# BDMstudio/audio-cut

Measured on AMD Instinct MI355X. Metric: audio-seconds processed/sec (separate+detect) per GPU; cut-point index parity, higher is better.
Workload: dtype f32

## Files before the change

### audio_cut_amd/csrc/ac_gemm.hip

```cpp
#include "ac_common.h"
#include "../../include/audiocut_hip_final.h"

typedef __attribute__((ext_vector_type(8))) _Float16 f16x8;
typedef __attribute__((ext_vector_type(4))) float f32x4;

#define GM_BM 128
#define GM_BM_FINAL 96
#define GM_BK 32
#define GM_ASTRIDE 48

__device__ inline unsigned short gm_f16_bits(_Float16 h) { return __builtin_bit_cast(unsigned short, h); }

template <int NT, bool RESID, int BM = GM_BM, int TR = 8, bool FINAL = false>
__global__ __launch_bounds__(256, 2) void k_tdf_linear_f16x3(const float* __restrict__ x, const f16x8* __restrict__ wpk,
                                                             const float* __restrict__ scale, const float* __restrict__ shift,
                                                             const float* __restrict__ resid, float* __restrict__ y,
                                                             int n_mblk, int N, int K, int T, int C, float w_unscale,
                                                             const float* __restrict__ in_amax, float* __restrict__ out_amax,
                                                             int ord_g, int ord_r, const float* __restrict__ fin_w = nullptr,
                                                             const float* __restrict__ fin_b = nullptr, float* __restrict__ spec = nullptr,
                                                             int C_out = 0) {
    static_assert(FINAL ? (BM == 96 && NT == 6 && RESID) : (BM == 128 && TR == 8), "row tiles: 16 channels x 8 time rows, or 48 x 2 with the final 1x1 conv");
    constexpr int MT = BM / 32;
    constexpr int A_ITERS = (BM * (GM_BK / 4)) / 256;
    constexpr int CH = BM / TR;
    constexpr int BN = 32 * NT;
    constexpr int BFRAGS = 2 * (BN / 16) * 64;
    constexpr int B_ITERS = BFRAGS / 256;
    constexpr int OSTRIDE = 16 * NT + 4;
    constexpr int A_BYTES = 2 * BM * GM_ASTRIDE * 2;
    constexpr int O_BYTES = 4 * 16 * OSTRIDE * 4;
    constexpr int TSTRIDE = BN + 4;
    constexpr int K_ARENA = A_BYTES + 2 * BFRAGS * 16, E_ARENA = FINAL ? BM * TSTRIDE * 4 : O_BYTES;
    constexpr int ARENA = K_ARENA > E_ARENA ? K_ARENA : E_ARENA;
    __shared__ __attribute__((aligned(16))) unsigned char s_raw[ARENA];
    unsigned short* s_hi = reinterpret_cast<unsigned short*>(s_raw);
    unsigned short* s_lo = s_hi + BM * GM_ASTRIDE;
    f16x8* s_b0 = reinterpret_cast<f16x8*>(s_raw + A_BYTES);
    f16x8* s_b1 = s_b0 + BFRAGS;
    float* s_out = reinterpret_cast<float*>(s_raw);

    const int tid = threadIdx.x, lane = tid & 63, wave = tid >> 6;
    const int wm = wave >> 1, wn = wave & 1;
    const int n_nblk = N / BN;
    int wi = blockIdx.x;
    if ((gridDim.x & 7) == 0) wi = (blockIdx.x & 7) * (gridDim.x >> 3) + (blockIdx.x >> 3);
    const int per = ord_r * n_nblk;
    const int chunk = wi / per, i_in = wi - chunk * per;
    const int nb_hi = i_in / (ord_g * ord_r), j_in = i_in - nb_hi * (ord_g * ord_r);
    const int nb = nb_hi * ord_g + j_in % ord_g, mb = chunk * ord_r + j_in / ord_g;
    if (mb >= n_mblk) return;
    const int n0 = nb * BN;
    const int n_stage = K / GM_BK;
    const int n_blk = T / TR, n_cg = C / CH;
    const int tb = mb % n_blk, cg = (mb / n_blk) % n_cg, item = mb / (n_blk * n_cg);
    const size_t m_base = ((size_t)item * C + (size_t)cg * CH) * T + (size_t)tb * TR;
    auto grow = [&](int r) -> size_t { return m_base + (size_t)(r / TR) * T + (r % TR); };
    __shared__ float s_scale[TR], s_inv[TR];
    __shared__ unsigned s_tmax[TR];
    if (tid < TR) {
        float inv;
        s_scale[tid] = ac_act_scale_lane(in_amax ? in_amax + (size_t)item * T : nullptr, tb * TR + tid, tb * TR + tid, &inv);
        s_inv[tid] = inv;
        s_tmax[tid] = 0u;
    }

    f32x4 acc[MT][NT];
#pragma unroll
    for (int m = 0; m < MT; ++m)
#pragma unroll
        for (int n = 0; n < NT; ++n) acc[m][n] = (f32x4){0.f, 0.f, 0.f, 0.f};

    const float* a_ptr[A_ITERS];
    int a_off[A_ITERS];
#pragma unroll
    for (int i = 0; i < A_ITERS; ++i) {
        const int e = tid + 256 * i;
        const int row = e >> 3, kq = e & 7;
        a_ptr[i] = x + grow(row) * (size_t)K + 4 * kq;
        a_off[i] = row * GM_ASTRIDE + 4 * kq;
    }
    const f16x8* wbase = wpk + (size_t)nb * n_stage * BFRAGS;

    float4 pre_a[A_ITERS];
    auto prefetch = [&](int s) {
        f16x8* dst = (s & 1) ? s_b1 : s_b0;
#pragma unroll
        for (int i = 0; i < B_ITERS; ++i) {
            const int inst = wave + 4 * i;
            __builtin_amdgcn_global_load_lds(wbase + (size_t)s * BFRAGS + inst * 64 + lane, dst + inst * 64, 16, 0, 0);
        }
#pragma unroll
        for (int i = 0; i < A_ITERS; ++i) pre_a[i] = *reinterpret_cast<const float4*>(a_ptr[i] + (size_t)s * GM_BK);
    };
    prefetch(0);
    __syncthreads();
    float a_scale[A_ITERS];
#pragma unroll
    for (int i = 0; i < A_ITERS; ++i) a_scale[i] = s_scale[((tid + 256 * i) >> 3) % TR];

    const int frag_row = lane & 15, frag_k = 8 * (lane >> 4);
    for (int s = 0; s < n_stage; ++s) {
        __syncthreads();
        const f16x8* s_b = (s & 1) ? s_b1 : s_b0;
#pragma unroll
        for (int i = 0; i < A_ITERS; ++i) {
            const float v[4] = {pre_a[i].x, pre_a[i].y, pre_a[i].z, pre_a[i].w};
            unsigned short h[4], l[4];
#pragma unroll
            for (int q = 0; q < 4; ++q) {
                const float c = fminf(fmaxf(v[q] * a_scale[i], -65504.f), 65504.f);
                const _Float16 hv = (_Float16)c;
                h[q] = gm_f16_bits(hv);
                l[q] = gm_f16_bits((_Float16)(c - (float)hv));
            }
            *reinterpret_cast<uint2*>(&s_hi[a_off[i]]) = make_uint2((unsigned)h[0] | ((unsigned)h[1] << 16), (unsigned)h[2] | ((unsigned)h[3] << 16));
            *reinterpret_cast<uint2*>(&s_lo[a_off[i]]) = make_uint2((unsigned)l[0] | ((unsigned)l[1] << 16), (unsigned)l[2] | ((unsigned)l[3] << 16));
        }
        __builtin_amdgcn_s_waitcnt(0);
        __syncthreads();
        if (s + 1 < n_stage) prefetch(s + 1);
        f16x8 ah[MT], al[MT];
#pragma unroll
        for (int m = 0; m < MT; ++m) {
            const int off = (wm * (BM / 2) + m * 16 + frag_row) * GM_ASTRIDE + frag_k;
            ah[m] = *reinterpret_cast<const f16x8*>(&s_hi[off]);
            al[m] = *reinterpret_cast<const f16x8*>(&s_lo[off]);
        }
#pragma unroll
        for (int n = 0; n < NT; ++n) {
            const f16x8 bh = s_b[(0 * (BN / 16) + wn * NT + n) * 64 + lane];
            const f16x8 bl = s_b[(1 * (BN / 16) + wn * NT + n) * 64 + lane];
#pragma unroll
            for (int m = 0; m < MT; ++m) {
                acc[m][n] = __builtin_amdgcn_mfma_f32_16x16x32_f16(ah[m], bl, acc[m][n], 0, 0, 0);
                acc[m][n] = __builtin_amdgcn_mfma_f32_16x16x32_f16(al[m], bh, acc[m][n], 0, 0, 0);
                acc[m][n] = __builtin_amdgcn_mfma_f32_16x16x32_f16(ah[m], bh, acc[m][n], 0, 0, 0);
            }
        }
    }
    if constexpr (FINAL) {
        constexpr int WR = BM / 2, WC = BN / 2;
        constexpr int ROW_F4 = WC / 4;
        constexpr int P_ITERS = 16 * ROW_F4 / 64;
        const int g = lane >> 4, px = lane & 15;
        float* s_tile = reinterpret_cast<float*>(s_raw);
        float* sw = s_tile + wm * WR * TSTRIDE + wn * WC;
        auto y_offset = [&](int m, int i, int& tr) -> size_t {
            const int e = lane + 64 * i;
            const int row = e / ROW_F4, q4 = e - row * ROW_F4;
            tr = wm * WR + m * 16 + row;
            return grow(tr) * (size_t)N + n0 + wn * WC + 4 * q4;
        };
        float4 rr[2][P_ITERS];
#pragma unroll
        for (int i = 0; i < P_ITERS; ++i) { int tr; rr[0][i] = *reinterpret_cast<const float4*>(resid + y_offset(0, i, tr)); }
        __syncthreads();
#pragma unroll
        for (int m = 0; m < MT; ++m)
#pragma unroll
            for (int n = 0; n < NT; ++n)
#pragma unroll
                for (int r = 0; r < 4; ++r) sw[(m * 16 + g * 4 + r) * TSTRIDE + n * 16 + px] = acc[m][n][r];
        __builtin_amdgcn_wave_barrier();
#pragma unroll
        for (int m = 0; m < MT; ++m) {
            if (m + 1 < MT) {
#pragma unroll
                for (int i = 0; i < P_ITERS; ++i) { int tr; rr[(m + 1) & 1][i] = *reinterpret_cast<const float4*>(resid + y_offset(m + 1, i, tr)); }
            }
#pragma unroll
            for (int i = 0; i < P_ITERS; ++i) {
                const int e = lane + 64 * i;
                const int row = e / ROW_F4, q4 = e - row * ROW_F4;
                int tr;
                const size_t o = y_offset(m, i, tr);
                const int c = cg * CH + tr / TR;
                const float sc = scale[c] * (w_unscale * s_inv[tr % TR]), sh = shift[c];
                float4* cell = reinterpret_cast<float4*>(&sw[(m * 16 + row) * TSTRIDE + 4 * q4]);
                float4 v = *cell;
                v.x = fmaxf(v.x * sc + sh, 0.f); v.y = fmaxf(v.y * sc + sh, 0.f);
                v.z = fmaxf(v.z * sc + sh, 0.f); v.w = fmaxf(v.w * sc + sh, 0.f);
                const float4 q = rr[m & 1][i];
                v.x += q.x; v.y += q.y; v.z += q.z; v.w += q.w;
                *cell = v;
                if (y) *reinterpret_cast<float4*>(y + o) = v;
            }
        }
        __syncthreads();
        if (tid < TR * (BN / 2)) {
            const int t = tid / (BN / 2), cp = tid - t * (BN / 2);
            const float* tp = s_tile + t * TSTRIDE + 2 * cp;
            int cw[4];
            float2 a[4];
#pragma unroll
            for (int co = 0; co < 4; ++co) {
                cw[co] = co < C_out ? co : 0;
                const float bv = fin_b[cw[co]];
                a[co] = make_float2(bv, bv);
            }
#pragma unroll
            for (int c = 0; c < CH; ++c) {
                const float2 v = *reinterpret_cast<const float2*>(tp + c * TR * TSTRIDE);
#pragma unroll
                for (int co = 0; co < 4; ++co) {
                    const float wv = fin_w[cw[co] * CH + c];
                    a[co].x = fmaf(wv, v.x, a[co].x); a[co].y = fmaf(wv, v.y, a[co].y);
                }
            }
#pragma unroll
            for (int co = 0; co < 4; ++co)
                if (co < C_out)
                    *reinterpret_cast<float2*>(spec + (((size_t)item * C_out + co) * T + (size_t)tb * TR + t) * N + n0 + 2 * cp) = a[co];
        }
        return;
    }
    const int g = lane >> 4, px = lane & 15;
    float* so = s_out + wave * 16 * OSTRIDE;
    constexpr int ROW_F4 = 4 * NT;
    constexpr int E_ITERS = 16 * ROW_F4 / 64;
    float4 rr[2][E_ITERS];
    auto out_offset = [&](int m, int i, int& c) -> size_t {
        const int e = lane + 64 * i;
        const int row = e / ROW_F4, q4 = e - row * ROW_F4;
        const int tr = wm * 64 + m * 16 + row;
        c = cg * 16 + (tr >> 3);
        return grow(tr) * (size_t)N + n0 + wn * (16 * NT) + 4 * q4;
    };
    if (RESID) {
#pragma unroll
        for (int i = 0; i < E_ITERS; ++i) { int c; rr[0][i] = *reinterpret_cast<const float4*>(resid + out_offset(0, i, c)); }
    }
    __syncthreads();
    float vm[E_ITERS];
#pragma unroll
    for (int i = 0; i < E_ITERS; ++i) vm[i] = 0.f;
#pragma unroll
    for (int m = 0; m < MT; ++m) {
#pragma unroll
        for (int n = 0; n < NT; ++n)
#pragma unroll
            for (int r = 0; r < 4; ++r) so[(g * 4 + r) * OSTRIDE + n * 16 + px] = acc[m][n][r];
        if (RESID && m + 1 < MT) {
#pragma unroll
            for (int i = 0; i < E_ITERS; ++i) { int c; rr[(m + 1) & 1][i] = *reinterpret_cast<const float4*>(resid + out_offset(m + 1, i, c)); }
        }
        __builtin_amdgcn_wave_barrier();
#pragma unroll
        for (int i = 0; i < E_ITERS; ++i) {
            const int e = lane + 64 * i;
            const int row = e / ROW_F4, q4 = e - row * ROW_F4;
            int c;
            const size_t o = out_offset(m, i, c);
            const int tr = wm * 64 + m * 16 + row;
            const float sc = scale[c] * (w_unscale * s_inv[tr & 7]), sh = shift[c];
            float4 v = *reinterpret_cast<const float4*>(&so[row * OSTRIDE + 4 * q4]);
            v.x = fmaxf(v.x * sc + sh, 0.f); v.y = fmaxf(v.y * sc + sh, 0.f);
            v.z = fmaxf(v.z * sc + sh, 0.f); v.w = fmaxf(v.w * sc + sh, 0.f);
            if (RESID) { const float4 q = rr[m & 1][i]; v.x += q.x; v.y += q.y; v.z += q.z; v.w += q.w; }
            vm[i] = fmaxf(fmaxf(vm[i], fmaxf(fabsf(v.x), fabsf(v.y))), fmaxf(fabsf(v.z), fabsf(v.w)));
            *reinterpret_cast<float4*>(y + o) = v;
        }
        __builtin_amdgcn_wave_barrier();
    }
    if (out_amax) {
#pragma unroll
        for (int i = 0; i < E_ITERS; ++i) {
            float a = fmaxf(vm[i], __shfl_xor(vm[i], 1, AC_WAVE));
            a = fmaxf(a, __shfl_xor(a, 2, AC_WAVE));
            if ((lane & 3) == 0) atomicMax(&s_tmax[((lane + 64 * i) / ROW_F4) & 7], __float_as_uint(a));
        }
        __syncthreads();
        if (tid < 8 && s_tmax[tid]) atomicMax(reinterpret_cast<unsigned*>(out_amax + (size_t)item * T + tb * 8 + tid), s_tmax[tid]);
    }
}

extern "C" int ac_tdf_linear_f16x3(ac_ctx* ctx, const float* x, const void* w_packed, const float* scale, const float* shift,
                                    const float* resid, float* y, long long M, int N, int K, int T, int C, float w_unscale,
                                    const float* in_amax, float* out_amax, void* stream) {
    AC_REQUIRE(ctx && x && w_packed && scale && shift && y, "null pointer");
    AC_REQUIRE(M > 0 && C > 0 && T > 0 && C % 16 == 0 && T % 8 == 0 && M % ((long long)C * T) == 0,
               "rows = items x C x T with C % 16 == 0 and T % 8 == 0 (a tile is 16 channels x 8 time rows)");
    AC_REQUIRE(K > 0 && K % GM_BK == 0, "K % 32 == 0");
    AC_REQUIRE(N > 0 && N % 96 == 0, "N % 96 == 0");
    const bool wide = (N % 192) == 0;
    const long long n_mblk = M / GM_BM;
    const int n_nblk = N / (wide ? 192 : 96);
    long long nblk = n_mblk * n_nblk;
    AC_REQUIRE(nblk < (1LL << 31) - 8 && n_mblk < (1LL << 31), "grid too large");
    int ord_g = n_nblk, ord_r = 1;
    if (n_nblk % 4 == 0 && n_nblk > 4 && n_mblk % 16 == 0) { ord_g = 4; ord_r = 16; }
    dim3 grid((unsigned)nblk), block(256);
    hipStream_t st = (hipStream_t)stream;
    const f16x8* wp = (const f16x8*)w_packed;
#define GM_GO(NT_, RES_) hipLaunchKernelGGL((k_tdf_linear_f16x3<NT_, RES_>), grid, block, 0, st, x, wp, scale, shift, resid, y, (int)n_mblk, N, K, T, C, w_unscale, in_amax, out_amax, ord_g, ord_r)
    if (wide) { if (resid) GM_GO(6, true); else GM_GO(6, false); }
    else      { if (resid) GM_GO(3, true); else GM_GO(3, false); }
#undef GM_GO
    AC_LAUNCH_CHECK();
    return AC_OK;
}

extern "C" int ac_tdf_linear_final_f16x3(ac_ctx* ctx, const float* x, const void* w_packed, const float* scale, const float* shift,
                                          const float* resid, const float* final_w, const float* final_b, float* spec, float* y,
                                          long long M, int N, int K, int T, int C, int C_out, float w_unscale, const float* in_amax,
                                          void* stream) {
    AC_REQUIRE(ctx && x && w_packed && scale && shift && spec, "null pointer");
    AC_REQUIRE(resid, "the residual is required (this is the block's second TDF layer)");
    AC_REQUIRE(final_w && final_b, "null pointer (final conv)");
    AC_REQUIRE(C > 0 && GM_BM_FINAL % C == 0, "96 % C == 0 (a tile holds every channel of its pixels)");
    AC_REQUIRE(C == 48, "C == 48 (the tile built is 48 channels x 2 time rows)");
    AC_REQUIRE(T > 0 && T % (GM_BM_FINAL / C) == 0, "T % (96 / C) == 0");
    AC_REQUIRE(M > 0 && M % ((long long)C * T) == 0, "rows = items x C x T");
    AC_REQUIRE(N > 0 && N % 192 == 0, "N % 192 == 0");
    AC_REQUIRE(K > 0 && K % GM_BK == 0, "K % 32 == 0");
    AC_REQUIRE(C_out >= 1 && C_out <= 4, "1 <= C_out <= 4");
    const long long n_mblk = M / GM_BM_FINAL;
    const int n_nblk = N / 192;
    const long long nblk = n_mblk * n_nblk;
    AC_REQUIRE(nblk < (1LL << 31) - 8 && n_mblk < (1LL << 31), "grid too large");
    int ord_g = n_nblk, ord_r = 1;
    if (n_nblk % 4 == 0 && n_nblk > 4 && n_mblk % 16 == 0) { ord_g = 4; ord_r = 16; }
    dim3 grid((unsigned)nblk), block(256);
    hipLaunchKernelGGL((k_tdf_linear_f16x3<6, true, GM_BM_FINAL, 2, true>), grid, block, 0, (hipStream_t)stream, x, (const f16x8*)w_packed,
                       scale, shift, resid, y, (int)n_mblk, N, K, T, C, w_unscale, in_amax, (float*)nullptr, ord_g, ord_r, final_w, final_b,
                       spec, C_out);
    AC_LAUNCH_CHECK();
    return AC_OK;
}
```

Before: 1496.

## Apply final epilogue in registers and split final 1x1 conv across all four waves

The FINAL epilogue now applies scale, shift, ReLU and the residual directly to the accumulator registers in MFMA fragment layout. It then writes the results to shared memory and y with scalar stores, instead of first spilling raw accumulators and re-reading them as float4. The final 1x1 conv, which used only 192 of 256 threads for all four output channels, is split so three waves each compute three channels for 64 slots and the fourth wave computes channel 3 for all 192 slots. This is meant to balance work across waves and drop a shared-memory round trip. The cost is scalar (non-vector) loads and stores for resid and y.

```diff
diff --git a/audio_cut_amd/csrc/ac_gemm.hip b/audio_cut_amd/csrc/ac_gemm.hip
--- a/audio_cut_amd/csrc/ac_gemm.hip
+++ b/audio_cut_amd/csrc/ac_gemm.hip
@@ -1,3 +1,5 @@
+#include <type_traits>
+
 #include "ac_common.h"
 #include "../../include/audiocut_hip_final.h"
 
@@ -141,78 +143,89 @@
     }
     if constexpr (FINAL) {
         constexpr int WR = BM / 2, WC = BN / 2;
-        constexpr int ROW_F4 = WC / 4;
-        constexpr int P_ITERS = 16 * ROW_F4 / 64;
         const int g = lane >> 4, px = lane & 15;
         float* s_tile = reinterpret_cast<float*>(s_raw);
-        float* sw = s_tile + wm * WR * TSTRIDE + wn * WC;
-        auto y_offset = [&](int m, int i, int& tr) -> size_t {
-            const int e = lane + 64 * i;
-            const int row = e / ROW_F4, q4 = e - row * ROW_F4;
-            tr = wm * WR + m * 16 + row;
-            return grow(tr) * (size_t)N + n0 + wn * WC + 4 * q4;
-        };
-        float4 rr[2][P_ITERS];
-#pragma unroll
-        for (int i = 0; i < P_ITERS; ++i) { int tr; rr[0][i] = *reinterpret_cast<const float4*>(resid + y_offset(0, i, tr)); }
-        __syncthreads();
-#pragma unroll
-        for (int m = 0; m < MT; ++m)
-#pragma unroll
-            for (int n = 0; n < NT; ++n)
-#pragma unroll
-                for (int r = 0; r < 4; ++r) sw[(m * 16 + g * 4 + r) * TSTRIDE + n * 16 + px] = acc[m][n][r];
-        __builtin_amdgcn_wave_barrier();
+        float* sw = s_tile + (wm * WR + g * 4) * TSTRIDE + wn * WC + px;
+        auto y_offset = [&](int m, int r) -> size_t { return grow(wm * WR + m * 16 + g * 4 + r) * (size_t)N + n0 + wn * WC + px; };
+        float rr[2][4][NT];
+#pragma unroll
+        for (int r = 0; r < 4; ++r)
+#pragma unroll
+            for (int n = 0; n < NT; ++n) rr[0][r][n] = resid[y_offset(0, r) + n * 16];
+        __syncthreads();
 #pragma unroll
         for (int m = 0; m < MT; ++m) {
             if (m + 1 < MT) {
 #pragma unroll
-                for (int i = 0; i < P_ITERS; ++i) { int tr; rr[(m + 1) & 1][i] = *reinterpret_cast<const float4*>(resid + y_offset(m + 1, i, tr)); }
-            }
-#pragma unroll
-            for (int i = 0; i < P_ITERS; ++i) {
-                const int e = lane + 64 * i;
-                const int row = e / ROW_F4, q4 = e - row * ROW_F4;
-                int tr;
-                const size_t o = y_offset(m, i, tr);
+                for (int r = 0; r < 4; ++r)
+#pragma unroll
+                    for (int n = 0; n < NT; ++n) rr[(m + 1) & 1][r][n] = resid[y_offset(m + 1, r) + n * 16];
+            }
+#pragma unroll
+            for (int r = 0; r < 4; ++r) {
+                const int tr = wm * WR + m * 16 + g * 4 + r;
                 const int c = cg * CH + tr / TR;
                 const float sc = scale[c] * (w_unscale * s_inv[tr % TR]), sh = shift[c];
-                float4* cell = reinterpret_cast<float4*>(&sw[(m * 16 + row) * TSTRIDE + 4 * q4]);
-                float4 v = *cell;
-                v.x = fmaxf(v.x * sc + sh, 0.f); v.y = fmaxf(v.y * sc + sh, 0.f);
-                v.z = fmaxf(v.z * sc + sh, 0.f); v.w = fmaxf(v.w * sc + sh, 0.f);
-                const float4 q = rr[m & 1][i];
-                v.x += q.x; v.y += q.y; v.z += q.z; v.w += q.w;
-                *cell = v;
-                if (y) *reinterpret_cast<float4*>(y + o) = v;
-            }
-        }
-        __syncthreads();
-        if (tid < TR * (BN / 2)) {
-            const int t = tid / (BN / 2), cp = tid - t * (BN / 2);
-            const float* tp = s_tile + t * TSTRIDE + 2 * cp;
-            int cw[4];
-            float2 a[4];
-#pragma unroll
-            for (int co = 0; co < 4; ++co) {
-                cw[co] = co < C_out ? co : 0;
-                const float bv = fin_b[cw[co]];
-                a[co] = make_float2(bv, bv);
+#pragma unroll
+                for (int n = 0; n < NT; ++n) {
+                    acc[m][n][r] = fmaxf(acc[m][n][r] * sc + sh, 0.f) + rr[m & 1][r][n];
+                    sw[(m * 16 + r) * TSTRIDE + n * 16] = acc[m][n][r];
+                }
+            }
+            if (y) {
+#pragma unroll
+                for (int r = 0; r < 4; ++r)
+#pragma unroll
+                    for (int n = 0; n < NT; ++n) y[y_offset(m, r) + n * 16] = acc[m][n][r];
+            }
+        }
+        __syncthreads();
+        static_assert(TR * (BN / 2) == 192, "three waves of slots, one output channel left for the fourth wave");
+        auto chain = [&](auto ns, auto nco, int s0, int co0) {
+            constexpr int NS = decltype(ns)::value, NCO = decltype(nco)::value;
+            const float* tp[NS];
+            size_t so[NS];
+#pragma unroll
+            for (int i = 0; i < NS; ++i) {
+                const int s = s0 + 64 * i;
+                const int t = s / (BN / 2), cp = s - t * (BN / 2);
+                tp[i] = s_tile + t * TSTRIDE + 2 * cp;
+                so[i] = ((size_t)tb * TR + t) * N + n0 + 2 * cp;
+            }
+            int cw[NCO];
+            float2 a[NS][NCO];
+#pragma unroll
+            for (int k = 0; k < NCO; ++k) {
+                cw[k] = co0 + k < C_out ? co0 + k : 0;
+                const float bv = fin_b[cw[k]];
+#pragma unroll
+                for (int i = 0; i < NS; ++i) a[i][k] = make_float2(bv, bv);
             }
 #pragma unroll
             for (int c = 0; c < CH; ++c) {
-                const float2 v = *reinterpret_cast<const float2*>(tp + c * TR * TSTRIDE);
-#pragma unroll
-                for (int co = 0; co < 4; ++co) {
-                    const float wv = fin_w[cw[co] * CH + c];
-                    a[co].x = fmaf(wv, v.x, a[co].x); a[co].y = fmaf(wv, v.y, a[co].y);
+                float2 v[NS];
+#pragma unroll
+                for (int i = 0; i < NS; ++i) v[i] = *reinterpret_cast<const float2*>(tp[i] + c * TR * TSTRIDE);
+#pragma unroll
+                for (int k = 0; k < NCO; ++k) {
+                    const float wv = fin_w[cw[k] * CH + c];
+#pragma unroll
+                    for (int i = 0; i < NS; ++i) { a[i][k].x = fmaf(wv, v[i].x, a[i][k].x); a[i][k].y = fmaf(wv, v[i].y, a[i][k].y); }
                 }
             }
 #pragma unroll
-            for (int co = 0; co < 4; ++co)
-                if (co < C_out)
-                    *reinterpret_cast<float2*>(spec + (((size_t)item * C_out + co) * T + (size_t)tb * TR + t) * N + n0 + 2 * cp) = a[co];
-        }
+            for (int k = 0; k < NCO; ++k)
+                if (co0 + k < C_out) {
+#pragma unroll
+                    for (int i = 0; i < NS; ++i)
+                        *reinterpret_cast<float2*>(spec + ((size_t)item * C_out + co0 + k) * T * N + so[i]) = a[i][k];
+                }
+        };
+        using one = std::integral_constant<int, 1>;
+        using three = std::integral_constant<int, 3>;
+        const int uw = __builtin_amdgcn_readfirstlane(wave);
+        if (uw < 3) chain(one{}, three{}, 64 * uw + lane, 0);
+        else if (C_out > 3) chain(three{}, one{}, lane, 3);
         return;
     }
     const int g = lane >> 4, px = lane & 15;
```

New measurement: 1500, median of 5. About the same (+0.3%).
